# rapidsai/cudf

Hardware: NVIDIA H100
Metric: sort_by_key_rows_per_s (higher is better)
Workload: dtype int64

## Files before the change

### cudf_b200/csrc/radix_sort.cu

```cuda
#include "common.cuh"
#include "device_utils.cuh"

#include <algorithm>
#include <cmath>
#include <cstdlib>
#include <type_traits>

namespace b2 {
namespace {

constexpr int RADIX_BITS = 8;
constexpr int RADIX      = 256;
constexpr uint32_t FLAG_AGG  = 1u << 30;
constexpr uint32_t FLAG_INCL = 2u << 30;
constexpr uint32_t VAL_MASK  = (1u << 30) - 1;

struct pass_plan {
  int32_t trivial;
  int32_t key_src;
  int32_t key_dst;
  int32_t idx_src;
  int32_t idx_dst;
  int32_t last;
  int32_t hybrid;
// ... 289 lines not shown
  const void* key_bufs[3];
  int32_t* idx_bufs[3];
  sort_ctl* ctl;
  uint32_t* status;
  uint32_t* tile_counter;
  int64_t portion_start;
  uint32_t portion_n;
  int32_t pass;
  int32_t portion_parity;
  int32_t has_next_portion;
  int32_t kind;
  int32_t pairs;
  uint64_t desc_mask;
  int32_t keep_keys;
  const void* val_in;
  const void* range_splitters;
  void* const* range_key_dst;
  void* const* range_val_dst;
  int32_t range_parts;
  int32_t range_hash;
  uint32_t est_cap;
};

__host__ __device__ __forceinline__ unsigned range_hash_bucket(uint64_t twiddled_key, int parts)
{
  const uint64_t h = mix64(twiddled_key + 0x9E3779B97F4A7C15ull);
  return (unsigned)(((h >> 32) * (uint64_t)parts) >> 32);
}

__device__ __forceinline__ void cta_barrier(int nthreads)
{
// ... 117 lines not shown
               : "memory");
#else
  (void)mbar;
#endif
}

template <int THREADS, int IPT, int MIN_BLOCKS, bool BULK = false>
struct tile_shape {
  static constexpr int threads = THREADS, ipt = IPT, min_blocks = MIN_BLOCKS, tile = THREADS * IPT;
  static constexpr bool bulk = BULK;
};
using tile_384x16      = tile_shape<384, 16, 2>;
using tile_512x16      = tile_shape<512, 16, 1>;
using tile_512x20_bulk = tile_shape<512, 20, 1, true>;

template <typename UK, typename Shape, typename VT, bool CARRY, bool MIX, bool RANGE>
__global__ void __launch_bounds__(Shape::threads + 32 * LBW, Shape::min_blocks) onesweep_kernel(pass_args a)
{
  constexpr int THREADS = Shape::threads;
  constexpr int IPT     = Shape::ipt;
  constexpr bool BULK   = Shape::bulk;
  constexpr int TILE    = THREADS * IPT;
  constexpr int NWARPS = THREADS / 32;
  static_assert(THREADS >= RADIX, "need one ranking thread per digit");
  static_assert(!RANGE || (!MIX && !BULK), "the range-partition pass uses the plain key load");

  const pass_plan pl = a.ctl->plan[a.pass];
  if (pl.trivial) return;

  B2_DYNAMIC_SMEM(smem_raw);
  constexpr int STAGE_W = sizeof(UK) > sizeof(VT) ? sizeof(UK) : sizeof(VT);
// ... 2 lines not shown
  uint32_t* s_whist   = reinterpret_cast<uint32_t*>(smem_raw + (size_t)STAGE_W * TILE);
  uint32_t* s_bm      = s_whist + NWARPS * RADIX;
  uint32_t* s_off     = s_bm + NWARPS * RADIX;
  uint32_t* s_cnt     = s_off + RADIX;
  uint32_t* s_misc    = s_cnt + 2 * RADIX;
  UK* s_split         = reinterpret_cast<UK*>(s_misc + 16);
  void** s_kdst       = reinterpret_cast<void**>(s_split + RADIX);
  void** s_vdst       = s_kdst + RADIX;
  uint8_t* s_dig      = reinterpret_cast<uint8_t*>(s_vdst + RADIX);

  const int tid  = threadIdx.x;
  const int lane = tid & 31;
  const int warp = tid >> 5;
  const bool ranker = warp < NWARPS;

  if (tid == 0) s_misc[0] = atomicAdd(a.tile_counter, 1u);
  if constexpr (BULK && !EMU_BUILD) {
    if (tid == 0) mbar_init_one((uint32_t)__cvta_generic_to_shared(s_misc + 12));
  }
  if (ranker) {
#pragma unroll
    for (int j = 0; j < RADIX / 32; ++j) {
      s_whist[warp * RADIX + j * 32 + lane] = 0;
      s_bm[warp * RADIX + j * 32 + lane]    = 0;
    }
  }
  if constexpr (RANGE) {
    for (int i = tid; i < RADIX; i += THREADS + 32 * LBW) {
      s_split[i] = (!a.range_hash && i < a.range_parts - 1) ? static_cast<const UK*>(a.range_splitters)[i] : ~UK(0);
      s_kdst[i]  = i < a.range_parts ? a.range_key_dst[i] : nullptr;
      s_vdst[i]  = (CARRY && i < a.range_parts) ? a.range_val_dst[i] : nullptr;
    }
  }
  __syncthreads();
  const uint32_t tile = s_misc[0];
  const uint32_t tile_base = tile * (uint32_t)TILE;
  const uint32_t tile_n = min((uint32_t)TILE, a.portion_n - tile_base);
  const bool full = tile_n == (uint32_t)TILE;
  const uint32_t pad = (uint32_t)TILE - tile_n;
  const int shift = a.pass * RADIX_BITS;
  const UK desc = (UK)a.desc_mask;

  if (!ranker) {
    cta_barrier(THREADS + 32 * LBW);
    const int d0 = ((warp - NWARPS) * 32 + lane) * DPL;
    uint32_t cnt[DPL], loc[DPL], excl[DPL];
#pragma unroll
    for (int j = 0; j < DPL; j += 2) {
      const uint4 cs = *reinterpret_cast<const uint4*>(s_cnt + 2 * (d0 + j));
      cnt[j] = cs.x; loc[j] = cs.y; cnt[j + 1] = cs.z; loc[j + 1] = cs.w;
      excl[j] = 0; excl[j + 1] = 0;
    }
// ... 32 lines not shown
        const int n_ready   = __ffs(~usable) - 1;
        const int first_inc = (inc_all & usable) ? (__ffs(inc_all & usable) - 1) : LBT;
        const int take = min(n_ready, first_inc + 1);
        if (take == 0) { __nanosleep(40); continue; }
#pragma unroll
        for (int r = 0; r < LBT; ++r) {
          if (r < take) { excl[0] += v[r].x & VAL_MASK; excl[1] += v[r].y; excl[2] += v[r].z; excl[3] += v[r].w; }
        }
        done = first_inc < n_ready;
        t -= take;
      }
      publish(FLAG_INCL, excl[0] + cnt[0], excl[1] + cnt[1], excl[2] + cnt[2], excl[3] + cnt[3]);
    }
    const uint32_t* gb = &a.ctl->base[a.portion_parity][a.pass][d0];
    bool wants_end = a.has_next_portion != 0;
    if constexpr (MIX) wants_end = wants_end || a.est_cap != 0u;
    const bool last_of_portion = wants_end && tile_base + tile_n == a.portion_n;
#pragma unroll
    for (int j = 0; j < DPL; ++j) {
      const uint32_t g = gb[j];
      s_off[d0 + j] = g + excl[j] - loc[j];
      if (last_of_portion) a.ctl->base[a.portion_parity ^ 1][a.pass][d0 + j] = g + excl[j] + cnt[j];
    }
    cta_barrier(THREADS + 32 * LBW);
    return;
  }

  UK key[IPT];
  const uint32_t wbase = tile_base + warp * (32 * IPT) + lane;
  {
    const UK* src = static_cast<const UK*>(pl.key_src == 0 ? a.key_bufs[0] : (pl.key_src == 1 ? a.key_bufs[1] : a.key_bufs[2])) + a.portion_start;
    bool via_smem = false;
// ... 8 lines not shown
        } else {
          const uint32_t mbar = (uint32_t)__cvta_generic_to_shared(s_misc + 12);
          if (tid == 0) bulk_copy_to_smem(s_keys, src + tile_base, BYTES, mbar);
          mbar_wait_phase0(mbar);
        }
#pragma unroll
        for (int i = 0; i < IPT; ++i) key[i] = s_keys[warp * (32 * IPT) + i * 32 + lane];
      }
    } else if (full) {
#pragma unroll
      for (int i = 0; i < IPT; ++i) key[i] = ld_stream(src + wbase + i * 32);
    } else {
#pragma unroll
      for (int i = 0; i < IPT; ++i) {
        uint32_t e = wbase + i * 32;
        key[i] = e < a.portion_n ? ld_stream(src + e) : UK(0);
      }
    }
    if (pl.key_src == 0) {
#pragma unroll
      for (int i = 0; i < IPT; ++i) {
        if constexpr (MIX) key[i] = (UK)mix64((uint64_t)key[i]);
        else key[i] = twiddle_rt<UK>(key[i], a.kind, desc);
      }
    }
    if (!full) {
#pragma unroll
      for (int i = 0; i < IPT; ++i)
        if (wbase + i * 32 >= a.portion_n) key[i] = ~UK(0);
    }
  }

  auto digit_of = [&](UK k) -> unsigned {
    if constexpr (RANGE) {
      if (a.range_hash) return range_hash_bucket((uint64_t)k, a.range_parts);
      int lo = 0, hi = a.range_parts - 1;
      while (lo < hi) {
        const int mid = (lo + hi) >> 1;
        if (s_split[mid] <= k) lo = mid + 1;
        else hi = mid;
      }
      return (unsigned)lo;
    } else {
      return (unsigned)(k >> shift) & 255u;
    }
  };
  unsigned dg[RANGE ? IPT : 1];
  if constexpr (RANGE) {
#pragma unroll
    for (int i = 0; i < IPT; ++i) dg[i] = (wbase + i * 32 >= a.portion_n) ? (unsigned)(RADIX - 1) : digit_of(key[i]);
  }
  auto digit_at = [&](int i) -> unsigned {
    if constexpr (RANGE) return dg[i];
    else return (unsigned)(key[i] >> shift) & 255u;
  };
  uint32_t* my_hist = s_whist + warp * RADIX;
  const int distinct = warp_digit_counts<IPT>(digit_at, IPT, lane, my_hist);
  ranker_barrier(THREADS);

  uint32_t tstart = 0, count = 0;
  if (tid < RADIX) {
#pragma unroll
    for (int w = 0; w < NWARPS; ++w) {
      uint32_t c = s_whist[w * RADIX + tid];
      s_whist[w * RADIX + tid] = count;
      count += c;
    }
    const uint32_t padded = count;
    if (tid == RADIX - 1) count -= pad;
    uint32_t inc = warp_inclusive_sum(padded);
    if (lane == 31) s_misc[1 + warp] = inc;
    tstart = inc - padded;
  }
// ... 14 lines not shown
  warp_rank<IPT>(digit_at, IPT, distinct, lane, my_hist, s_bm + warp * RADIX, pos);
#pragma unroll
  for (int i = 0; i < IPT; ++i) s_keys[pos[i]] = key[i];
  if constexpr (RANGE) {
#pragma unroll
    for (int i = 0; i < IPT; ++i) s_dig[pos[i]] = (uint8_t)dg[i];
  }
  VT idx[IPT];
  if (a.pairs) {
    if (pl.idx_src < 0) {
      if constexpr (CARRY) {
        const VT* vsrc = static_cast<const VT*>(a.val_in) + a.portion_start;
#pragma unroll
        for (int i = 0; i < IPT; ++i) {
          const uint32_t e = wbase + i * 32;
          idx[i] = e < a.portion_n ? ld_stream(vsrc + e) : VT(0);
        }
      } else {
#pragma unroll
        for (int i = 0; i < IPT; ++i) idx[i] = (uint32_t)(a.portion_start + wbase + i * 32);
      }
    } else {
      const VT* isrc = reinterpret_cast<const VT*>(pl.idx_src == 0 ? a.idx_bufs[0] : (pl.idx_src == 1 ? a.idx_bufs[1] : a.idx_bufs[2])) + a.portion_start;
      if (full) {
#pragma unroll
        for (int i = 0; i < IPT; ++i) idx[i] = ld_stream(isrc + wbase + i * 32);
      } else {
#pragma unroll
        for (int i = 0; i < IPT; ++i) {
          uint32_t e = wbase + i * 32;
          idx[i] = e < a.portion_n ? ld_stream(isrc + e) : VT(0);
        }
      }
    }
  }
  cta_barrier(THREADS + 32 * LBW);

  const bool write_keys = !(a.pairs && pl.last) || a.keep_keys || pl.hybrid;
  UK* kdst = static_cast<UK*>(const_cast<void*>(pl.key_dst == 1 ? a.key_bufs[1] : a.key_bufs[2]));
  uint32_t dst[IPT];
  uint8_t dstd[RANGE ? IPT : 1];
#pragma unroll
  for (int j = 0; j < IPT; ++j) {
    const uint32_t q = j * THREADS + tid;
    UK k = s_keys[q];
    unsigned d;
    if constexpr (RANGE) d = s_dig[q];
    else d = (unsigned)(k >> shift) & 255u;
    dst[j] = s_off[d] + q;
    if constexpr (MIX) {
      if (a.est_cap != 0u && dst[j] >= (d + 1u) * a.est_cap) {
        if (q < tile_n) a.ctl->overflow = 1u;
        dst[j] = 0xFFFFFFFFu;
      }
    }
    if constexpr (RANGE) {
      dstd[j] = (uint8_t)d;
      if (q < tile_n) static_cast<UK*>(s_kdst[d])[dst[j]] = untwiddle_rt<UK>(k, a.kind, desc);
    } else if (write_keys && q < tile_n && (!MIX || dst[j] != 0xFFFFFFFFu)) {
      if (!a.pairs && pl.last && !pl.hybrid) k = untwiddle_rt<UK>(k, a.kind, desc);
      kdst[dst[j]] = k;
    }
  }
  if (a.pairs) {
    ranker_barrier(THREADS);
#pragma unroll
    for (int i = 0; i < IPT; ++i) s_vals[pos[i]] = idx[i];
    ranker_barrier(THREADS);
    VT* idst = reinterpret_cast<VT*>(pl.idx_dst == 0 ? a.idx_bufs[0] : (pl.idx_dst == 1 ? a.idx_bufs[1] : a.idx_bufs[2]));
#pragma unroll
    for (int j = 0; j < IPT; ++j) {
      const uint32_t q = j * THREADS + tid;
      if constexpr (RANGE) {
        if (q < tile_n) static_cast<VT*>(s_vdst[dstd[j]])[dst[j]] = s_vals[q];
      } else {
        if (q < tile_n && (!MIX || dst[j] != 0xFFFFFFFFu)) idst[dst[j]] = s_vals[q];
      }
    }
  }
}

template <typename UK, bool MIX = false>
__global__ void finalize_kernel(pass_args a, int64_t n, int raw, int pre_idx_buf, int carry_bytes)
{
  if (a.ctl->any_pass != 0) return;
  if (carry_bytes) {
    const int64_t stride = (int64_t)gridDim.x * blockDim.x;
    for (int64_t i = (int64_t)blockIdx.x * blockDim.x + threadIdx.x; i < n; i += stride) {
      if (carry_bytes == 8) reinterpret_cast<uint64_t*>(a.idx_bufs[0])[i] = static_cast<const uint64_t*>(a.val_in)[i];
      else reinterpret_cast<uint32_t*>(a.idx_bufs[0])[i] = static_cast<const uint32_t*>(a.val_in)[i];
      if (a.keep_keys && raw) {
// ... 153 lines not shown
  const bool bulk = (reinterpret_cast<uintptr_t>(g) % sizeof(T)) == 0 && s >= off && m + off >= PER;
  const int bulk_rows = bulk ? (m + off) / PER * PER : 0;
  if (bulk) {
    if constexpr (EMU_BUILD) {
      for (int q = threadIdx.x; q < bulk_rows; q += RANGE_THREADS) sdst[q] = g[q - off];
    } else {
      if (threadIdx.x == 0) bulk_copy_to_smem(sdst, g - off, (uint32_t)(sizeof(T) * bulk_rows), mbar);
    }
    for (int r = bulk_rows - off + (int)threadIdx.x; r < m; r += RANGE_THREADS) sdst[off + r] = g[r];
  } else {
    for (int q = threadIdx.x; q < m; q += RANGE_THREADS) sdst[q] = ld_stream(g + q);
  }
  return {bulk ? off : 0, bulk};
}

template <typename VT>
__global__ void __launch_bounds__(RANGE_THREADS, 1) range_sort_kernel(pass_args a, const uint32_t* __restrict__ bounds)
{
  using UK = uint64_t;
  B2_DYNAMIC_SMEM(smem_raw);
  uint32_t* s_misc = reinterpret_cast<uint32_t*>(smem_raw);
  UK* s_keys       = reinterpret_cast<UK*>(smem_raw + 128);
  VT* s_vals       = reinterpret_cast<VT*>(s_keys);
  uint32_t* s_cnt  = reinterpret_cast<uint32_t*>(s_keys + RANGE_CAP + 2);
  uint16_t* s_perm = reinterpret_cast<uint16_t*>(s_cnt + RANGE_BUCKETS);

  const int tid = threadIdx.x, lane = tid & 31, warp = tid >> 5;
  const int64_t s = bounds[blockIdx.x];
  const int m = (int)(bounds[blockIdx.x + 1] - s);
  if (m == 0) return;
  if (m > RANGE_CAP) {
    if (tid == 0) atomicOr(&a.ctl->overflow, 1u);
    return;
  }
  const UK* __restrict__ keys = static_cast<const UK*>(a.ctl->fix_key_buf == 1 ? a.key_bufs[1] : a.key_bufs[2]) + s;
  const VT* __restrict__ vin  = reinterpret_cast<const VT*>(a.ctl->fix_idx_buf == 1 ? a.idx_bufs[1] : a.idx_bufs[2]) + s;
  VT* __restrict__ vout = reinterpret_cast<VT*>(a.idx_bufs[0]) + s;
  UK* __restrict__ kout = static_cast<UK*>(const_cast<void*>(a.key_bufs[1])) + s;

  const uint64_t below = a.ctl->vary & ((1ull << a.ctl->range_shift) - 1);
  const uint32_t vhi = (uint32_t)(below >> 32), vlo = (uint32_t)below;
  const int top = vhi ? 64 - __clz((int)vhi) : (vlo ? 32 - __clz((int)vlo) : 0);
  const int want = m > 1 ? 32 - __clz(m - 1) : 0;
  const int nb = min(min(want, RANGE_BUCKET_BITS), top);
  const int bshift = top - nb;
  const uint32_t bmask = (1u << nb) - 1;
  const int lp = max(nb - 9, 0);
  const int per = 1 << lp;
  auto bucket = [&](UK k) { return (uint32_t)(k >> bshift) & bmask; };
  auto slot   = [&](uint32_t b) { return ((b & (uint32_t)(per - 1)) << 9) | (b >> lp); };

  const uint32_t mbar_k = EMU_BUILD ? 0u : (uint32_t)__cvta_generic_to_shared(s_misc);
  const uint32_t mbar_v = EMU_BUILD ? 0u : (uint32_t)__cvta_generic_to_shared(s_misc + 2);
// ... 198 lines not shown
    }
  }
}

int64_t portion_rows(int tile)
{
  static const int64_t lim = [] {
    const char* e = std::getenv("B2_SORT_PORTION");
    int64_t v = e ? std::atoll(e) : 0;
    if (v <= 0) v = (int64_t(1) << 30) - 16384;
    return v;
  }();
  return std::max<int64_t>(tile, lim / tile * tile);
}

template <typename UK, typename Shape, typename VT, bool CARRY, bool MIX, bool RANGE = false>
struct onesweep_passes {
  static constexpr int TILE = Shape::tile;
  static constexpr size_t SMEM = (sizeof(UK) > sizeof(VT) ? sizeof(UK) : sizeof(VT)) * (size_t)TILE +
                                 sizeof(uint32_t) * (2 * (Shape::threads / 32) * RADIX + 3 * RADIX + 16) +
                                 (RANGE ? (sizeof(UK) + 2 * sizeof(void*)) * RADIX + (size_t)TILE : 0);
  static constexpr size_t CTL_BYTES = (sizeof(sort_ctl) + 255) / 256 * 256;
  const int64_t n, plim, nportions;
  const size_t hist_bytes, cnt_bytes, head_bytes, status_per;
  dbuf work;

  onesweep_passes(int64_t rows, int passes, size_t hist, size_t tail_bytes, cudaStream_t stream)
    : n(rows), plim(portion_rows(TILE)), nportions((n + plim - 1) / plim), hist_bytes(hist),
      cnt_bytes((sizeof(uint32_t) * passes * nportions + 255) / 256 * 256), head_bytes(CTL_BYTES + hist_bytes + cnt_bytes + tail_bytes),
      status_per(sizeof(uint32_t) * RADIX * (size_t)((std::min(n, plim) + TILE - 1) / TILE)),
      work(head_bytes + status_per * passes * nportions, stream)
  {
    static std::atomic<uint64_t> attr_done{0};
    once_per_device(attr_done, [] {
      B2_CUDA_TRY(cudaFuncSetAttribute(onesweep_kernel<UK, Shape, VT, CARRY, MIX, RANGE>, cudaFuncAttributeMaxDynamicSharedMemorySize, (int)SMEM));
    });
  }
  sort_ctl* ctl() const { return work.as<sort_ctl>(); }
  uint32_t* hist() const { return reinterpret_cast<uint32_t*>(work.as<char>() + CTL_BYTES); }
  void* tail() const { return work.as<char>() + CTL_BYTES + hist_bytes + cnt_bytes; }
  void zero_head(cudaStream_t stream) const { B2_CUDA_TRY(cudaMemsetAsync(work.ptr, 0, head_bytes, stream)); }

  void run(pass_args& a, int slot, const char* scope, cudaStream_t stream) const
  {
    for (int64_t q = 0; q < nportions; ++q) {
      const int64_t start = q * plim;
      const int64_t pn = std::min(plim, n - start);
      const int64_t ntiles = (pn + TILE - 1) / TILE;
      a.portion_start = start;
      a.portion_n = (uint32_t)pn;
      a.portion_parity = (int)(q & 1);
      a.has_next_portion = q + 1 < nportions;
      a.status = reinterpret_cast<uint32_t*>(work.as<char>() + head_bytes + (size_t)(slot * nportions + q) * status_per);
      a.tile_counter = reinterpret_cast<uint32_t*>(work.as<char>() + CTL_BYTES + hist_bytes) + slot * nportions + q;
      B2_CUDA_TRY(cudaMemsetAsync(a.status, 0, sizeof(uint32_t) * RADIX * (size_t)ntiles, stream));
      prof_scope ps(scope, stream);
      B2_LAUNCH((onesweep_kernel<UK, Shape, VT, CARRY, MIX, RANGE>), (unsigned)ntiles, Shape::threads + 32 * LBW, SMEM, stream, a);
    }
  }
};

constexpr int64_t RANGE_MIN_ROWS = int64_t(1) << 27;
int range_env()
{
  static int v = [] {
    const char* e = std::getenv("B2_SORT_RANGE");
    return e ? (std::atoi(e) != 0 ? 1 : 0) : -1;
  }();
  return v;
}

int64_t hybrid_min_rows()
{
  static int64_t v = [] {
    const char* off = std::getenv("B2_SORT_HYBRID");
    if (off && std::atoi(off) == 0) return INT64_MAX;
    const char* e = std::getenv("B2_SORT_HYBRID_MIN");
    return e ? (int64_t)std::atoll(e) : (int64_t(1) << 16);
  }();
  return v;
}

template <typename UK, typename Shape, typename VT = uint32_t, bool CARRY = false, bool MIX = false>
void run_radix_cfg(const UK* raw_keys, UK* bufA, UK* bufB, int32_t* idx_out, int32_t* idx_tmp, int32_t* idx_tmp2, int pre_idx_buf, int64_t n,
                   int kind, bool descending, bool pairs, cudaStream_t stream, int first_pass = 0, int last_pass = 7,
                   bool keep_keys = false, const void* val_in = nullptr, uint32_t* top_digit_base_out = nullptr)
{
  constexpr int NP = sizeof(UK);
  const bool raw = raw_keys != nullptr;
  const UK desc_mask = descending ? ~UK(0) : UK(0);

  const onesweep_passes<UK, Shape, VT, CARRY, MIX> passes(n, NP, sizeof(uint32_t) * NP * RADIX, 0, stream);
  sort_ctl* const ctl = passes.ctl();
  uint32_t* const ghist = passes.hist();
  if constexpr (sizeof(UK) == 8 && !MIX) {
    static std::atomic<uint64_t> attr_done{0};
    once_per_device(attr_done, [] {
      B2_CUDA_TRY(cudaFuncSetAttribute(range_sort_kernel<VT>, cudaFuncAttributeMaxDynamicSharedMemorySize, (int)range_sort_smem()));
    });
  }

  bool try_hybrid = sizeof(UK) == 8 && !MIX && raw && first_pass == 0 && last_pass >= NP - 1 && !keep_keys && n >= hybrid_min_rows();
  const int force_range = range_env();
  bool try_range = try_hybrid && force_range != 0 && (force_range == 1 || n >= RANGE_MIN_ROWS);

// ... 107 lines not shown
    }
    try_hybrid = false;
  }
  if (pairs && raw && kind == (int)key_kind::FLOAT && descending) {
    B2_LAUNCH(reverse_nan_prefix_kernel, num_sms() * 4, 256, 0, stream, idx_out, &ctl->nan_count);
  }
  if (top_digit_base_out)
    B2_CUDA_TRY(cudaMemcpyAsync(top_digit_base_out, &ctl->base[0][NP - 1][0], sizeof(uint32_t) * RADIX, cudaMemcpyDeviceToDevice, stream));
}

template <typename UK>
using key_tile = std::conditional_t<sizeof(UK) == 8, tile_384x16, tile_512x16>;

template <typename UK>
void run_radix(const UK* raw_keys, UK* bufA, UK* bufB, int32_t* idx_out, int32_t* idx_tmp, int pre_idx_buf, int64_t n,
               int kind, bool descending, bool pairs, cudaStream_t stream, int32_t* idx_tmp2 = nullptr)
{
  run_radix_cfg<UK, key_tile<UK>>(raw_keys, bufA, bufB, idx_out, idx_tmp, idx_tmp2, pre_idx_buf, n, kind, descending, pairs, stream);
}

template void run_radix_cfg<uint64_t, tile_384x16>(const uint64_t*, uint64_t*, uint64_t*, int32_t*, int32_t*, int32_t*, int, int64_t, int, bool,
                                                   bool, cudaStream_t, int, int, bool, const void*, uint32_t*);

}

void radix_partition_top16_mix(const uint64_t* packed_keys, int64_t n, uint64_t* keys_out, int32_t* idx_out, cudaStream_t stream)
{
  dbuf b(sizeof(uint64_t) * n, stream), it(sizeof(int32_t) * n, stream);
  run_radix_cfg<uint64_t, tile_384x16, uint32_t, false, true>(packed_keys, keys_out, b.as<uint64_t>(), idx_out, it.as<int32_t>(), nullptr, 0,
                                                              n, (int)key_kind::UNSIGNED, false, true, stream, 6, 7, true);
}

void radix_partition_mix_carry(const uint64_t* keys, const void* vals, int val_bytes, int64_t n, uint64_t* mixed_keys_out, void* vals_out,
                               uint32_t* part_base, cudaStream_t stream)
{
  dbuf b(sizeof(uint64_t) * n, stream), vt((size_t)val_bytes * n, stream);
  if (val_bytes == 8)
// ... 19 lines not shown
      pl.idx_src = -1;
      pl.key_dst = 1;
      pl.idx_dst = 0;
      pl.last    = 1;
      pl.hybrid  = 0;
    }
    ctl->plan[d] = pl;
  }
  if (d == 0) {
    ctl->any_pass = 1;
    ctl->hybrid   = 0;
    ctl->overflow = 0;
  }
}

__global__ void __launch_bounds__(256) est_sample_kernel(const uint64_t* __restrict__ keys, int64_t n, int64_t stride, unsigned int* __restrict__ counts)
{
  __shared__ unsigned int sh[RADIX];
  sh[threadIdx.x] = 0;
  __syncthreads();
  const int64_t m = (n + stride - 1) / stride;
  for (int64_t i = (int64_t)blockIdx.x * blockDim.x + threadIdx.x; i < m; i += (int64_t)gridDim.x * blockDim.x)
    atomicAdd(&sh[(unsigned)(mix64(keys[i * stride]) >> 56)], 1u);
  __syncthreads();
  if (sh[threadIdx.x]) atomicAdd(&counts[threadIdx.x], sh[threadIdx.x]);
}

template <typename VT>
bool est_pass_impl(const uint64_t* keys, const void* vals, int64_t n, uint32_t cap, uint64_t* mixed_keys_out, void* vals_out, uint32_t* part_base,
                   uint32_t* part_end, cudaStream_t stream)
{
  constexpr int PASS = 7;
  const onesweep_passes<uint64_t, tile_384x16, VT, true, true> passes(n, 1, 0, 0, stream);
  sort_ctl* const ctl = passes.ctl();
  passes.zero_head(stream);
  B2_LAUNCH(est_plan_kernel, 1, RADIX, 0, stream, ctl, PASS, cap);
  pass_args a{};
  a.key_bufs[0] = keys;
  a.key_bufs[1] = mixed_keys_out;
  a.key_bufs[2] = mixed_keys_out;
// ... 19 lines not shown
}

uint32_t radix_partition_est_capacity(const uint64_t* keys, int64_t n, cudaStream_t stream)
{
  static const int64_t min_rows = [] {
    const char* e = std::getenv("B2_GROUPBY_EST_MIN");
    return e ? (int64_t)std::atoll(e) : (int64_t(1) << 22);
  }();
  if (n < min_rows || n > portion_rows(tile_384x16::tile)) return 0;
  if (const char* e = std::getenv("B2_GROUPBY_EST_CAP")) return (uint32_t)std::max(1, std::atoi(e));
  const int64_t want = int64_t(1) << 20;
  const int64_t stride = std::max<int64_t>(1, n / want);
  const int64_t m = (n + stride - 1) / stride;
  dbuf cnt(sizeof(unsigned int) * RADIX, stream);
  B2_CUDA_TRY(cudaMemsetAsync(cnt.ptr, 0, cnt.bytes, stream));
  B2_LAUNCH(est_sample_kernel, num_sms() * 4, 256, 0, stream, keys, n, stride, cnt.as<unsigned int>());
  unsigned int h[RADIX];
  B2_CUDA_TRY(cudaMemcpyAsync(h, cnt.ptr, sizeof(h), cudaMemcpyDeviceToHost, stream));
  B2_CUDA_TRY(cudaStreamSynchronize(stream));
  unsigned int mx = 0;
  for (int d = 0; d < RADIX; ++d) mx = std::max(mx, h[d]);
  const double cap = (double)(n / RADIX) * 1.25 + 4096.0;
  const double worst = ((double)mx + 5.0 * std::sqrt((double)mx) + 1.0) * ((double)n / (double)m);
  if (worst > cap || cap * RADIX >= 4.0e9) return 0;
  return (uint32_t)cap;
}

bool radix_partition_mix_carry_est(const uint64_t* keys, const void* vals, int val_bytes, int64_t n, uint32_t cap, uint64_t* mixed_keys_out,
                                   void* vals_out, uint32_t* part_base, uint32_t* part_end, cudaStream_t stream)
{
  if (val_bytes == 8) return est_pass_impl<uint64_t>(keys, vals, n, cap, mixed_keys_out, vals_out, part_base, part_end, stream);
// ... 96 lines not shown
}

void range_partition_scatter(const b2_column_view& keys, const b2_column_view* values, const void* splitters, int P, void* const* key_dst,
                             void* const* val_dst, cudaStream_t stream)
{
  if (keys.size == 0) return;
  if (values == nullptr) return range_scatter_impl<uint32_t, false>(keys, nullptr, splitters, P, key_dst, nullptr, stream);
  const int vw = type_width(values->type_id);
  const void* vin = static_cast<const char*>(values->data) + (size_t)values->offset * vw;
  if (vw == 8) range_scatter_impl<uint64_t, true>(keys, vin, splitters, P, key_dst, val_dst, stream);
  else range_scatter_impl<uint32_t, true>(keys, vin, splitters, P, key_dst, val_dst, stream);
}

namespace {

int kind_of(int32_t storage_id)
{
  if (is_float_id(storage_id)) return (int)key_kind::FLOAT;
  if (is_signed_id(storage_id)) return (int)key_kind::SIGNED;
  return (int)key_kind::UNSIGNED;
}

template <typename UK>
column_ptr sorted_order_single(const b2_column_view& col, bool ascending, bool nulls_before, cudaStream_t stream)
{
  const int64_t n = col.size;
  const int sid   = storage_type(col.type_id);
  const int kind  = kind_of(sid);
  auto out = make_column(B2_INT32, col.size, false, stream);
  const UK* data = static_cast<const UK*>(col.data) + col.offset;
  int32_t* out_idx = out->data.as<int32_t>();

  if (!has_nulls(col)) {
    dbuf a(sizeof(UK) * n, stream), b(sizeof(UK) > 1 ? sizeof(UK) * n : 0, stream), it(sizeof(int32_t) * n, stream);
    run_radix<UK>(data, a.as<UK>(), b.as<UK>(), out_idx, it.as<int32_t>(), 0, n, kind, !ascending, true, stream);
    return out;
  }
  const bool nulls_first = nulls_before != !ascending;
  const int64_t n_null  = col.null_count;
  const int64_t n_valid = n - n_null;
  const int64_t ntiles = (n + CP_ROWS - 1) / CP_ROWS;
  dbuf tv(sizeof(uint32_t) * (ntiles + 1), stream);
  B2_LAUNCH(valid_count_kernel, (unsigned)((ntiles + 7) / 8), CP_THREADS, 0, stream, col.null_mask, (int64_t)col.offset, n,
            tv.as<uint32_t>());
  B2_LAUNCH(scan_tiles_kernel, 1, 1024, 0, stream, tv.as<uint32_t>(), ntiles, tv.as<uint32_t>() + ntiles);
  dbuf a(sizeof(UK) * std::max<int64_t>(n_valid, 1), stream), b(sizeof(UK) * std::max<int64_t>(n_valid, 1), stream);
  dbuf it(sizeof(int32_t) * std::max<int64_t>(n_valid, 1), stream), it2(sizeof(int32_t) * std::max<int64_t>(n_valid, 1), stream);
  int32_t* valid_out = out_idx + (nulls_first ? n_null : 0);
  int32_t* null_out  = out_idx + (nulls_first ? 0 : n_valid);
  const UK desc_mask = ascending ? UK(0) : ~UK(0);
// ... 161 lines not shown
  return v;
}
bool sort_carry_applicable(const b2_column_view& keys, const b2_column_view& values, bool ascending)
{
  const int vw = type_width(values.type_id);
  const bool float_desc = is_float_id(storage_type(keys.type_id)) && !ascending;
  return sort_carry_enabled() && is_radix_sortable(keys) && !has_nulls(values) && (vw == 4 || vw == 8) && !float_desc &&
         keys.size == values.size && keys.size > 0;
}
column_ptr sort_by_key_carry(const b2_column_view& keys, const b2_column_view& values, bool ascending, cudaStream_t stream)
{
  const int64_t n = keys.size;
  const int kind = kind_of(storage_type(keys.type_id));
  auto out = make_column(values.type_id, (int32_t)n, false, stream);
  const int vw = type_width(values.type_id);
  dbuf vtmp((size_t)vw * n, stream);
  const void* vin = static_cast<const char*>(values.data) + (size_t)values.offset * vw;
  auto go = [&](auto ktag, auto vtag) {
    using UK = decltype(ktag);
    using VT = decltype(vtag);
    dbuf a(sizeof(UK) * n, stream), b(sizeof(UK) > 1 ? sizeof(UK) * n : 0, stream);
    using Shape = std::conditional_t<sizeof(UK) == 8 && sizeof(VT) == 8, tile_512x20_bulk, key_tile<UK>>;
    run_radix_cfg<UK, Shape, VT, true>(static_cast<const UK*>(keys.data) + keys.offset, a.as<UK>(), b.as<UK>(), out->data.as<int32_t>(),
                                       vtmp.as<int32_t>(), nullptr, 0, n, kind, !ascending, true, stream, 0, 7, false, vin);
  };
  auto by_key = [&](auto vtag) {
    switch (type_width(keys.type_id)) {
      case 1: go(uint8_t{}, vtag); break;
      case 2: go(uint16_t{}, vtag); break;
      case 4: go(uint32_t{}, vtag); break;
      default: go(uint64_t{}, vtag); break;
    }
  };
  if (vw == 8) by_key(uint64_t{}); else by_key(uint32_t{});
  return out;
}

column_ptr sort_single_column(const b2_column_view& col, bool ascending, cudaStream_t stream)
{
  const int64_t n = col.size;
  auto out = make_column(col.type_id, col.size, false, stream);
  if (n == 0) return out;
  const int kind = kind_of(storage_type(col.type_id));
  B2_EXPECTS(kind != (int)key_kind::FLOAT, B2_ERR_LOGIC, "keys-only radix path is for integer-like keys");
  auto run = [&](auto tag) {
    using UK = decltype(tag);
    dbuf tmp(sizeof(UK) > 1 ? sizeof(UK) * n : 0, stream);
    run_radix<UK>(static_cast<const UK*>(col.data) + col.offset, out->data.as<UK>(), tmp.as<UK>(), nullptr, nullptr, 0, n, kind,
                  !ascending, false, stream);
  };
  switch (type_width(col.type_id)) {
    case 1: run(uint8_t{}); break;
    case 2: run(uint16_t{}); break;
    case 4: run(uint32_t{}); break;
    case 8: run(uint64_t{}); break;
    default: B2_FAIL(B2_ERR_DATA_TYPE, "sort: unsupported key type");
  }
  return out;
}

}
```

Before: 22.72 billion.

## Add sampled-capacity two-pass MSD radix tier with range sort for 64-bit keys

Adds an estimated-capacity path for 64-bit keys. A sampling kernel builds histograms of the top two digits and picks a per-bucket capacity. Only the top two radix passes then run, scattering into padded fixed-offset buckets, and a range_sort kernel sorts each of the 65536 segments, replacing the six remaining onesweep passes. This costs extra memory (padded buffers), a host sync for sampling plus a later overflow check with fallback, and more kernels.

```diff
diff --git a/cudf_b200/csrc/radix_sort.cu b/cudf_b200/csrc/radix_sort.cu
--- a/cudf_b200/csrc/radix_sort.cu
+++ b/cudf_b200/csrc/radix_sort.cu
@@ -327,7 +327,10 @@
   uint64_t desc_mask;
   int32_t keep_keys;
   const void* val_in;
-  const void* range_splitters;
+  union {
+    const void* range_splitters;
+    const uint2* est_tiles;
+  };
   void* const* range_key_dst;
   void* const* range_val_dst;
   int32_t range_parts;
@@ -475,7 +478,7 @@
 using tile_512x16      = tile_shape<512, 16, 1>;
 using tile_512x20_bulk = tile_shape<512, 20, 1, true>;
 
-template <typename UK, typename Shape, typename VT, bool CARRY, bool MIX, bool RANGE>
+template <typename UK, typename Shape, typename VT, bool CARRY, bool MIX, bool RANGE, bool EST = false>
 __global__ void __launch_bounds__(Shape::threads + 32 * LBW, Shape::min_blocks) onesweep_kernel(pass_args a)
 {
   constexpr int THREADS = Shape::threads;
@@ -508,7 +511,19 @@
   const int warp = tid >> 5;
   const bool ranker = warp < NWARPS;
 
-  if (tid == 0) s_misc[0] = atomicAdd(a.tile_counter, 1u);
+  if (tid == 0) {
+    const uint32_t t = atomicAdd(a.tile_counter, 1u);
+    s_misc[0] = t;
+    if constexpr (EST) {
+      s_misc[10] = 0;
+      s_misc[11] = 0;
+      if (a.est_tiles != nullptr) {
+        const uint2 e = a.est_tiles[t];
+        s_misc[9]  = e.x;
+        s_misc[14] = e.y;
+      }
+    }
+  }
   if constexpr (BULK && !EMU_BUILD) {
     if (tid == 0) mbar_init_one((uint32_t)__cvta_generic_to_shared(s_misc + 12));
   }
@@ -528,8 +543,17 @@
   }
   __syncthreads();
   const uint32_t tile = s_misc[0];
-  const uint32_t tile_base = tile * (uint32_t)TILE;
-  const uint32_t tile_n = min((uint32_t)TILE, a.portion_n - tile_base);
+  uint32_t tile_base = tile * (uint32_t)TILE;
+  uint32_t tile_n = min((uint32_t)TILE, a.portion_n - tile_base);
+  uint32_t nlim = a.portion_n;
+  if constexpr (EST) {
+    if (a.est_tiles != nullptr) {
+      if (s_misc[14] == 0) return;
+      tile_base = s_misc[9];
+      tile_n    = s_misc[14] & 0x7fffffffu;
+      nlim      = tile_base + tile_n;
+    }
+  }
   const bool full = tile_n == (uint32_t)TILE;
   const uint32_t pad = (uint32_t)TILE - tile_n;
   const int shift = a.pass * RADIX_BITS;
@@ -592,8 +616,12 @@
     }
     const uint32_t* gb = &a.ctl->base[a.portion_parity][a.pass][d0];
     bool wants_end = a.has_next_portion != 0;
-    if constexpr (MIX) wants_end = wants_end || a.est_cap != 0u;
-    const bool last_of_portion = wants_end && tile_base + tile_n == a.portion_n;
+    if constexpr (MIX || EST) wants_end = wants_end || a.est_cap != 0u;
+    bool last_tile = tile_base + tile_n == a.portion_n;
+    if constexpr (EST) {
+      if (a.est_tiles != nullptr) last_tile = (s_misc[14] >> 31) != 0u;
+    }
+    const bool last_of_portion = wants_end && last_tile;
 #pragma unroll
     for (int j = 0; j < DPL; ++j) {
       const uint32_t g = gb[j];
@@ -632,7 +660,7 @@
 #pragma unroll
       for (int i = 0; i < IPT; ++i) {
         uint32_t e = wbase + i * 32;
-        key[i] = e < a.portion_n ? ld_stream(src + e) : UK(0);
+        key[i] = e < nlim ? ld_stream(src + e) : UK(0);
       }
     }
     if (pl.key_src == 0) {
@@ -645,7 +673,22 @@
     if (!full) {
 #pragma unroll
       for (int i = 0; i < IPT; ++i)
-        if (wbase + i * 32 >= a.portion_n) key[i] = ~UK(0);
+        if (wbase + i * 32 >= nlim) key[i] = ~UK(0);
+    }
+    if constexpr (EST) {
+      if (pl.key_src == 0) {
+        const UK k0 = twiddle_rt<UK>(static_cast<const UK*>(a.key_bufs[0])[0], a.kind, desc);
+        uint64_t v = 0;
+#pragma unroll
+        for (int i = 0; i < IPT; ++i)
+          if (wbase + i * 32 < nlim) v |= (uint64_t)(key[i] ^ k0);
+        const uint32_t lo = __reduce_or_sync(0xffffffffu, (uint32_t)v);
+        const uint32_t hi = __reduce_or_sync(0xffffffffu, (uint32_t)(v >> 32));
+        if (lane == 0 && (lo | hi)) {
+          atomicOr(&s_misc[10], lo);
+          atomicOr(&s_misc[11], hi);
+        }
+      }
     }
   }
 
@@ -666,7 +709,7 @@
   unsigned dg[RANGE ? IPT : 1];
   if constexpr (RANGE) {
 #pragma unroll
-    for (int i = 0; i < IPT; ++i) dg[i] = (wbase + i * 32 >= a.portion_n) ? (unsigned)(RADIX - 1) : digit_of(key[i]);
+    for (int i = 0; i < IPT; ++i) dg[i] = (wbase + i * 32 >= nlim) ? (unsigned)(RADIX - 1) : digit_of(key[i]);
   }
   auto digit_at = [&](int i) -> unsigned {
     if constexpr (RANGE) return dg[i];
@@ -675,6 +718,12 @@
   uint32_t* my_hist = s_whist + warp * RADIX;
   const int distinct = warp_digit_counts<IPT>(digit_at, IPT, lane, my_hist);
   ranker_barrier(THREADS);
+  if constexpr (EST) {
+    if (tid == 0 && pl.key_src == 0) {
+      const unsigned long long v = ((unsigned long long)s_misc[11] << 32) | s_misc[10];
+      if (v) atomicOr(&a.ctl->vary, v);
+    }
+  }
 
   uint32_t tstart = 0, count = 0;
   if (tid < RADIX) {
@@ -719,7 +768,7 @@
 #pragma unroll
         for (int i = 0; i < IPT; ++i) {
           const uint32_t e = wbase + i * 32;
-          idx[i] = e < a.portion_n ? ld_stream(vsrc + e) : VT(0);
+          idx[i] = e < nlim ? ld_stream(vsrc + e) : VT(0);
         }
       } else {
 #pragma unroll
@@ -734,7 +783,7 @@
 #pragma unroll
         for (int i = 0; i < IPT; ++i) {
           uint32_t e = wbase + i * 32;
-          idx[i] = e < a.portion_n ? ld_stream(isrc + e) : VT(0);
+          idx[i] = e < nlim ? ld_stream(isrc + e) : VT(0);
         }
       }
     }
@@ -753,7 +802,7 @@
     if constexpr (RANGE) d = s_dig[q];
     else d = (unsigned)(k >> shift) & 255u;
     dst[j] = s_off[d] + q;
-    if constexpr (MIX) {
+    if constexpr (MIX || EST) {
       if (a.est_cap != 0u && dst[j] >= (d + 1u) * a.est_cap) {
         if (q < tile_n) a.ctl->overflow = 1u;
         dst[j] = 0xFFFFFFFFu;
@@ -762,7 +811,7 @@
     if constexpr (RANGE) {
       dstd[j] = (uint8_t)d;
       if (q < tile_n) static_cast<UK*>(s_kdst[d])[dst[j]] = untwiddle_rt<UK>(k, a.kind, desc);
-    } else if (write_keys && q < tile_n && (!MIX || dst[j] != 0xFFFFFFFFu)) {
+    } else if (write_keys && q < tile_n && (!(MIX || EST) || dst[j] != 0xFFFFFFFFu)) {
       if (!a.pairs && pl.last && !pl.hybrid) k = untwiddle_rt<UK>(k, a.kind, desc);
       kdst[dst[j]] = k;
     }
@@ -779,7 +828,7 @@
       if constexpr (RANGE) {
         if (q < tile_n) static_cast<VT*>(s_vdst[dstd[j]])[dst[j]] = s_vals[q];
       } else {
-        if (q < tile_n && (!MIX || dst[j] != 0xFFFFFFFFu)) idst[dst[j]] = s_vals[q];
+        if (q < tile_n && (!(MIX || EST) || dst[j] != 0xFFFFFFFFu)) idst[dst[j]] = s_vals[q];
       }
     }
   }
@@ -963,7 +1012,36 @@
   return {bulk ? off : 0, bulk};
 }
 
-template <typename VT>
+__global__ void __launch_bounds__(RADIX) range_est_bounds_kernel(pass_args a, uint32_t cap, uint32_t* __restrict__ est)
+{
+  __shared__ uint32_t s_lb[RADIX + 1];
+  __shared__ uint32_t s_wsum[RADIX / 32];
+  constexpr int R = RADIX * RADIX;
+  const int d7 = blockIdx.x, d6 = threadIdx.x;
+  const uint64_t* __restrict__ keys = static_cast<const uint64_t*>(a.ctl->fix_key_buf == 1 ? a.key_bufs[1] : a.key_bufs[2]);
+  auto count = [&](int e) { return min(a.ctl->base[1][7][e] - (uint32_t)e * cap, cap); };
+  const uint32_t before = warp_sum(d6 < d7 ? count(d6) : 0u);
+  if ((d6 & 31) == 0) s_wsum[d6 >> 5] = before;
+  const uint32_t w0 = (uint32_t)d7 * cap, wn = count(d7);
+  uint32_t lo = 0, hi = wn;
+  while (lo < hi) {
+    const uint32_t mid = (lo + hi) >> 1;
+    if ((int)((keys[w0 + mid] >> 48) & 255u) < d6) lo = mid + 1;
+    else hi = mid;
+  }
+  s_lb[d6] = lo;
+  if (d6 == 0) s_lb[RADIX] = wn;
+  __syncthreads();
+  uint32_t dense = 0;
+  for (int w = 0; w < RADIX / 32; ++w) dense += s_wsum[w];
+  const uint32_t end = s_lb[d6 + 1];
+  const int i = d7 * RADIX + d6;
+  est[i]         = w0 + lo;
+  est[R + i]     = end > lo ? end - lo : 0u;
+  est[2 * R + i] = dense + lo;
+}
+
+template <typename VT, bool EST = false>
 __global__ void __launch_bounds__(RANGE_THREADS, 1) range_sort_kernel(pass_args a, const uint32_t* __restrict__ bounds)
 {
   using UK = uint64_t;
@@ -976,7 +1054,14 @@
 
   const int tid = threadIdx.x, lane = tid & 31, warp = tid >> 5;
   const int64_t s = bounds[blockIdx.x];
-  const int m = (int)(bounds[blockIdx.x + 1] - s);
+  int m;
+  int64_t o = s;
+  if constexpr (EST) {
+    m = (int)bounds[gridDim.x + blockIdx.x];
+    o = bounds[2 * gridDim.x + blockIdx.x];
+  } else {
+    m = (int)(bounds[blockIdx.x + 1] - s);
+  }
   if (m == 0) return;
   if (m > RANGE_CAP) {
     if (tid == 0) atomicOr(&a.ctl->overflow, 1u);
@@ -984,8 +1069,8 @@
   }
   const UK* __restrict__ keys = static_cast<const UK*>(a.ctl->fix_key_buf == 1 ? a.key_bufs[1] : a.key_bufs[2]) + s;
   const VT* __restrict__ vin  = reinterpret_cast<const VT*>(a.ctl->fix_idx_buf == 1 ? a.idx_bufs[1] : a.idx_bufs[2]) + s;
-  VT* __restrict__ vout = reinterpret_cast<VT*>(a.idx_bufs[0]) + s;
-  UK* __restrict__ kout = static_cast<UK*>(const_cast<void*>(a.key_bufs[1])) + s;
+  VT* __restrict__ vout = reinterpret_cast<VT*>(a.idx_bufs[0]) + o;
+  UK* __restrict__ kout = static_cast<UK*>(const_cast<void*>(a.key_bufs[1])) + o;
 
   const uint64_t below = a.ctl->vary & ((1ull << a.ctl->range_shift) - 1);
   const uint32_t vhi = (uint32_t)(below >> 32), vlo = (uint32_t)below;
@@ -1214,7 +1299,7 @@
   return std::max<int64_t>(tile, lim / tile * tile);
 }
 
-template <typename UK, typename Shape, typename VT, bool CARRY, bool MIX, bool RANGE = false>
+template <typename UK, typename Shape, typename VT, bool CARRY, bool MIX, bool RANGE = false, bool EST = false>
 struct onesweep_passes {
   static constexpr int TILE = Shape::tile;
   static constexpr size_t SMEM = (sizeof(UK) > sizeof(VT) ? sizeof(UK) : sizeof(VT)) * (size_t)TILE +
@@ -1225,15 +1310,16 @@
   const size_t hist_bytes, cnt_bytes, head_bytes, status_per;
   dbuf work;
 
-  onesweep_passes(int64_t rows, int passes, size_t hist, size_t tail_bytes, cudaStream_t stream)
+  onesweep_passes(int64_t rows, int passes, size_t hist, size_t tail_bytes, cudaStream_t stream, int extra_tiles = 0)
     : n(rows), plim(portion_rows(TILE)), nportions((n + plim - 1) / plim), hist_bytes(hist),
       cnt_bytes((sizeof(uint32_t) * passes * nportions + 255) / 256 * 256), head_bytes(CTL_BYTES + hist_bytes + cnt_bytes + tail_bytes),
-      status_per(sizeof(uint32_t) * RADIX * (size_t)((std::min(n, plim) + TILE - 1) / TILE)),
+      status_per(sizeof(uint32_t) * RADIX * (size_t)((std::min(n, plim) + TILE - 1) / TILE + extra_tiles)),
       work(head_bytes + status_per * passes * nportions, stream)
   {
     static std::atomic<uint64_t> attr_done{0};
     once_per_device(attr_done, [] {
-      B2_CUDA_TRY(cudaFuncSetAttribute(onesweep_kernel<UK, Shape, VT, CARRY, MIX, RANGE>, cudaFuncAttributeMaxDynamicSharedMemorySize, (int)SMEM));
+      B2_CUDA_TRY(cudaFuncSetAttribute(onesweep_kernel<UK, Shape, VT, CARRY, MIX, RANGE, EST>, cudaFuncAttributeMaxDynamicSharedMemorySize,
+                                       (int)SMEM));
     });
   }
   sort_ctl* ctl() const { return work.as<sort_ctl>(); }
@@ -1241,12 +1327,12 @@
   void* tail() const { return work.as<char>() + CTL_BYTES + hist_bytes + cnt_bytes; }
   void zero_head(cudaStream_t stream) const { B2_CUDA_TRY(cudaMemsetAsync(work.ptr, 0, head_bytes, stream)); }
 
-  void run(pass_args& a, int slot, const char* scope, cudaStream_t stream) const
+  void run(pass_args& a, int slot, const char* scope, cudaStream_t stream, int extra_tiles = 0) const
   {
     for (int64_t q = 0; q < nportions; ++q) {
       const int64_t start = q * plim;
       const int64_t pn = std::min(plim, n - start);
-      const int64_t ntiles = (pn + TILE - 1) / TILE;
+      const int64_t ntiles = (pn + TILE - 1) / TILE + extra_tiles;
       a.portion_start = start;
       a.portion_n = (uint32_t)pn;
       a.portion_parity = (int)(q & 1);
@@ -1255,7 +1341,7 @@
       a.tile_counter = reinterpret_cast<uint32_t*>(work.as<char>() + CTL_BYTES + hist_bytes) + slot * nportions + q;
       B2_CUDA_TRY(cudaMemsetAsync(a.status, 0, sizeof(uint32_t) * RADIX * (size_t)ntiles, stream));
       prof_scope ps(scope, stream);
-      B2_LAUNCH((onesweep_kernel<UK, Shape, VT, CARRY, MIX, RANGE>), (unsigned)ntiles, Shape::threads + 32 * LBW, SMEM, stream, a);
+      B2_LAUNCH((onesweep_kernel<UK, Shape, VT, CARRY, MIX, RANGE, EST>), (unsigned)ntiles, Shape::threads + 32 * LBW, SMEM, stream, a);
     }
   }
 };
@@ -1281,14 +1367,132 @@
   return v;
 }
 
+__global__ void range_est_plan_kernel(sort_ctl* ctl, uint32_t cap)
+{
+  const int d = threadIdx.x;
+  ctl->base[0][6][d] = (uint32_t)d * cap;
+  ctl->base[0][7][d] = (uint32_t)d * cap;
+  if (d < 8) {
+    pass_plan pl{};
+    pl.trivial = d < 6;
+    if (d >= 6) {
+      pl.key_src = d == 6 ? 0 : 1;
+      pl.key_dst = d == 6 ? 1 : 2;
+      pl.idx_src = d == 6 ? -1 : 2;
+      pl.idx_dst = d == 6 ? 2 : 1;
+      pl.last    = d == 7;
+      pl.hybrid  = 1;
+    }
+    ctl->plan[d] = pl;
+  }
+  if (d == 0) {
+    ctl->any_pass    = 2;
+    ctl->hybrid      = 1;
+    ctl->range       = 1;
+    ctl->range_shift = 48;
+    ctl->range_bits  = 16;
+    ctl->fix_shift   = 48;
+    ctl->fix_key_buf = 2;
+    ctl->fix_idx_buf = 1;
+    ctl->overflow    = 0;
+  }
+}
+
+__global__ void range_est_tiles_kernel(const sort_ctl* ctl, uint32_t cap, int tile, uint2* __restrict__ tiles)
+{
+  __shared__ uint32_t s_wsum[RADIX / 32];
+  const int d = threadIdx.x;
+  const uint32_t cnt = min(ctl->base[1][6][d] - (uint32_t)d * cap, cap);
+  const uint32_t nt = (cnt + (uint32_t)tile - 1) / (uint32_t)tile;
+  const uint32_t inc = warp_inclusive_sum(nt);
+  if ((d & 31) == 31) s_wsum[d >> 5] = inc;
+  __syncthreads();
+  uint32_t first = inc - nt, total = 0;
+  for (int w = 0; w < RADIX / 32; ++w) {
+    first += w < (d >> 5) ? s_wsum[w] : 0u;
+    total += s_wsum[w];
+  }
+  for (uint32_t k = 0; k < nt; ++k) {
+    const uint32_t off = k * (uint32_t)tile;
+    const uint32_t t = first + k;
+    tiles[t] = make_uint2((uint32_t)d * cap + off, min((uint32_t)tile, cnt - off) | (t + 1 == total ? 0x80000000u : 0u));
+  }
+}
+
+template <typename UK, typename Shape, typename VT, bool CARRY>
+bool run_est_range(const UK* raw_keys, UK* keys_out, UK* k1, UK* k2, int32_t* idx_out, int32_t* v1, int32_t* v2, int64_t n, uint32_t cap,
+                   int kind, UK desc_mask, bool pairs, const void* val_in, cudaStream_t stream)
+{
+  static_assert(sizeof(UK) == 8, "the estimated-base range tier sorts 64-bit keys");
+  constexpr int TILE = Shape::tile;
+  const int64_t ntiles = (n + TILE - 1) / TILE + RADIX;
+  const size_t table_bytes = (sizeof(uint2) * ntiles + 255) / 256 * 256;
+  const onesweep_passes<UK, Shape, VT, CARRY, false, false, true> passes(n, 2, 0, table_bytes, stream, RADIX);
+  {
+    static std::atomic<uint64_t> attr_done{0};
+    once_per_device(attr_done, [] {
+      B2_CUDA_TRY(cudaFuncSetAttribute(range_sort_kernel<VT, true>, cudaFuncAttributeMaxDynamicSharedMemorySize, (int)range_sort_smem()));
+    });
+  }
+  sort_ctl* const ctl = passes.ctl();
+  uint2* const tiles = static_cast<uint2*>(passes.tail());
+  passes.zero_head(stream);
+  B2_LAUNCH(range_est_plan_kernel, 1, RADIX, 0, stream, ctl, cap);
+  pass_args a{};
+  a.key_bufs[0] = raw_keys;
+  a.key_bufs[1] = k1;
+  a.key_bufs[2] = k2;
+  a.idx_bufs[0] = idx_out;
+  a.idx_bufs[1] = v2;
+  a.idx_bufs[2] = v1;
+  a.ctl = ctl;
+  a.kind = kind;
+  a.pairs = pairs ? 1 : 0;
+  a.val_in = val_in;
+  a.desc_mask = (uint64_t)desc_mask;
+  a.est_cap = cap;
+  a.pass = 6;
+  passes.run(a, 0, "onesweep", stream);
+  B2_LAUNCH(range_est_tiles_kernel, 1, RADIX, 0, stream, (const sort_ctl*)ctl, cap, TILE, tiles);
+  a.pass = 7;
+  a.est_tiles = tiles;
+  passes.run(a, 1, "onesweep", stream, RADIX);
+  a.key_bufs[1] = keys_out;
+  dbuf bounds(sizeof(uint32_t) * 3 * RADIX * RADIX, stream);
+  {
+    prof_scope ps("range_bounds", stream);
+    B2_LAUNCH(range_est_bounds_kernel, RADIX, RADIX, 0, stream, a, cap, bounds.as<uint32_t>());
+  }
+  {
+    prof_scope ps("segment_fix", stream);
+    B2_LAUNCH((range_sort_kernel<VT, true>), RADIX * RADIX, RANGE_THREADS, range_sort_smem(), stream, a, bounds.as<const uint32_t>());
+  }
+  uint32_t overflow = 0;
+  B2_CUDA_TRY(cudaMemcpyAsync(&overflow, &ctl->overflow, sizeof(overflow), cudaMemcpyDeviceToHost, stream));
+  B2_CUDA_TRY(cudaStreamSynchronize(stream));
+  return overflow == 0;
+}
+
 template <typename UK, typename Shape, typename VT = uint32_t, bool CARRY = false, bool MIX = false>
 void run_radix_cfg(const UK* raw_keys, UK* bufA, UK* bufB, int32_t* idx_out, int32_t* idx_tmp, int32_t* idx_tmp2, int pre_idx_buf, int64_t n,
                    int kind, bool descending, bool pairs, cudaStream_t stream, int first_pass = 0, int last_pass = 7,
-                   bool keep_keys = false, const void* val_in = nullptr, uint32_t* top_digit_base_out = nullptr)
+                   bool keep_keys = false, const void* val_in = nullptr, uint32_t* top_digit_base_out = nullptr, uint32_t est_cap = 0,
+                   void* est_buf = nullptr)
 {
   constexpr int NP = sizeof(UK);
   const bool raw = raw_keys != nullptr;
   const UK desc_mask = descending ? ~UK(0) : UK(0);
+
+  if constexpr (sizeof(UK) == 8 && !MIX) {
+    if (est_cap != 0 && raw && first_pass == 0 && last_pass >= NP - 1 && !keep_keys) {
+      const bool done =
+        pairs ? run_est_range<UK, Shape, VT, CARRY>(raw_keys, bufA, bufA, bufB, idx_out, static_cast<int32_t*>(est_buf), idx_tmp, n, est_cap,
+                                                    kind, desc_mask, true, val_in, stream)
+              : run_est_range<UK, Shape, VT, CARRY>(raw_keys, bufA, static_cast<UK*>(est_buf), bufB, nullptr, nullptr, nullptr, n, est_cap,
+                                                    kind, desc_mask, false, val_in, stream);
+      if (done) return;
+    }
+  }
 
   const onesweep_passes<UK, Shape, VT, CARRY, MIX> passes(n, NP, sizeof(uint32_t) * NP * RADIX, 0, stream);
   sort_ctl* const ctl = passes.ctl();
@@ -1426,13 +1630,15 @@
 
 template <typename UK>
 void run_radix(const UK* raw_keys, UK* bufA, UK* bufB, int32_t* idx_out, int32_t* idx_tmp, int pre_idx_buf, int64_t n,
-               int kind, bool descending, bool pairs, cudaStream_t stream, int32_t* idx_tmp2 = nullptr)
-{
-  run_radix_cfg<UK, key_tile<UK>>(raw_keys, bufA, bufB, idx_out, idx_tmp, idx_tmp2, pre_idx_buf, n, kind, descending, pairs, stream);
+               int kind, bool descending, bool pairs, cudaStream_t stream, int32_t* idx_tmp2 = nullptr, uint32_t est_cap = 0,
+               void* est_buf = nullptr)
+{
+  run_radix_cfg<UK, key_tile<UK>>(raw_keys, bufA, bufB, idx_out, idx_tmp, idx_tmp2, pre_idx_buf, n, kind, descending, pairs, stream, 0, 7,
+                                  false, nullptr, nullptr, est_cap, est_buf);
 }
 
 template void run_radix_cfg<uint64_t, tile_384x16>(const uint64_t*, uint64_t*, uint64_t*, int32_t*, int32_t*, int32_t*, int, int64_t, int, bool,
-                                                   bool, cudaStream_t, int, int, bool, const void*, uint32_t*);
+                                                   bool, cudaStream_t, int, int, bool, const void*, uint32_t*, uint32_t, void*);
 
 }
 
@@ -1482,16 +1688,27 @@
   }
 }
 
-__global__ void __launch_bounds__(256) est_sample_kernel(const uint64_t* __restrict__ keys, int64_t n, int64_t stride, unsigned int* __restrict__ counts)
-{
-  __shared__ unsigned int sh[RADIX];
-  sh[threadIdx.x] = 0;
+template <bool MIX = true>
+__global__ void __launch_bounds__(256) est_sample_kernel(const uint64_t* __restrict__ keys, int64_t n, int64_t stride, unsigned int* __restrict__ counts,
+                                                         int kind = 0, uint64_t desc_mask = 0)
+{
+  constexpr int NC = MIX ? 1 : 2;
+  __shared__ unsigned int sh[NC * RADIX];
+  for (int c = 0; c < NC; ++c) sh[c * RADIX + threadIdx.x] = 0;
   __syncthreads();
   const int64_t m = (n + stride - 1) / stride;
-  for (int64_t i = (int64_t)blockIdx.x * blockDim.x + threadIdx.x; i < m; i += (int64_t)gridDim.x * blockDim.x)
-    atomicAdd(&sh[(unsigned)(mix64(keys[i * stride]) >> 56)], 1u);
+  for (int64_t i = (int64_t)blockIdx.x * blockDim.x + threadIdx.x; i < m; i += (int64_t)gridDim.x * blockDim.x) {
+    if constexpr (MIX) {
+      atomicAdd(&sh[(unsigned)(mix64(keys[i * stride]) >> 56)], 1u);
+    } else {
+      const uint64_t k = twiddle_rt<uint64_t>(keys[i * stride], kind, desc_mask);
+      atomicAdd(&sh[(unsigned)(k >> 56)], 1u);
+      atomicAdd(&sh[RADIX + (unsigned)((k >> 48) & 255u)], 1u);
+    }
+  }
   __syncthreads();
-  if (sh[threadIdx.x]) atomicAdd(&counts[threadIdx.x], sh[threadIdx.x]);
+  for (int c = 0; c < NC; ++c)
+    if (sh[c * RADIX + threadIdx.x]) atomicAdd(&counts[c * RADIX + threadIdx.x], sh[c * RADIX + threadIdx.x]);
 }
 
 template <typename VT>
@@ -1541,7 +1758,7 @@
   const int64_t m = (n + stride - 1) / stride;
   dbuf cnt(sizeof(unsigned int) * RADIX, stream);
   B2_CUDA_TRY(cudaMemsetAsync(cnt.ptr, 0, cnt.bytes, stream));
-  B2_LAUNCH(est_sample_kernel, num_sms() * 4, 256, 0, stream, keys, n, stride, cnt.as<unsigned int>());
+  B2_LAUNCH((est_sample_kernel<true>), num_sms() * 4, 256, 0, stream, keys, n, stride, cnt.as<unsigned int>(), 0, (uint64_t)0);
   unsigned int h[RADIX];
   B2_CUDA_TRY(cudaMemcpyAsync(h, cnt.ptr, sizeof(h), cudaMemcpyDeviceToHost, stream));
   B2_CUDA_TRY(cudaStreamSynchronize(stream));
@@ -1668,6 +1885,60 @@
 
 namespace {
 
+int est_env()
+{
+  static int v = [] {
+    const char* e = std::getenv("B2_SORT_EST");
+    return e ? (std::atoi(e) != 0 ? 1 : 0) : -1;
+  }();
+  return v;
+}
+
+template <typename UK>
+uint32_t est_range_capacity(const UK* raw_keys, int64_t n, int kind, bool descending, bool pairs, int tile, cudaStream_t stream)
+{
+  if constexpr (sizeof(UK) != 8) {
+    return 0;
+  } else {
+    const int force = est_env();
+    if (force == 0 || n < 2 || n > portion_rows(tile)) return 0;
+    if (pairs && kind == (int)key_kind::FLOAT && descending) return 0;
+    if (range_env() == 0 || hybrid_min_rows() == INT64_MAX) return 0;
+    if (force != 1 && (n < RANGE_MIN_ROWS || n < hybrid_min_rows())) return 0;
+    if (const char* e = std::getenv("B2_SORT_EST_CAP")) return (uint32_t)std::max(1, std::atoi(e));
+    const int64_t stride = std::max<int64_t>(1, n >> 20);
+    const int64_t m = (n + stride - 1) / stride;
+    dbuf cnt(sizeof(unsigned int) * 2 * RADIX, stream);
+    B2_CUDA_TRY(cudaMemsetAsync(cnt.ptr, 0, cnt.bytes, stream));
+    {
+      prof_scope ps("est_sample", stream);
+      const int grid = (int)std::max<int64_t>(1, std::min<int64_t>((m + 255) / 256, num_sms() * 4));
+      B2_LAUNCH((est_sample_kernel<false>), grid, 256, 0, stream, reinterpret_cast<const uint64_t*>(raw_keys), n, stride, cnt.as<unsigned int>(),
+                kind, (uint64_t)(descending ? ~UK(0) : UK(0)));
+    }
+    unsigned int h[2 * RADIX];
+    B2_CUDA_TRY(cudaMemcpyAsync(h, cnt.ptr, sizeof(h), cudaMemcpyDeviceToHost, stream));
+    B2_CUDA_TRY(cudaStreamSynchronize(stream));
+    unsigned int mx[2] = {0, 0};
+    double coll[2] = {0.0, 0.0};
+    for (int c = 0; c < 2; ++c)
+      for (int d = 0; d < RADIX; ++d) {
+        mx[c] = std::max(mx[c], h[c * RADIX + d]);
+        const double f = (double)h[c * RADIX + d] / (double)m;
+        coll[c] += f * f;
+      }
+    if (mx[0] >= (unsigned)m || mx[1] >= (unsigned)m) return 0;
+    const double e = (double)n * coll[0] * coll[1];
+    if (e + 5.0 * std::sqrt(e) > (double)RANGE_CAP) return 0;
+    const double top = (double)std::max(mx[0], mx[1]);
+    const double worst = (top + 5.0 * std::sqrt(top) + 1.0) * ((double)n / (double)m);
+    if (worst > (double)(n / RADIX) * 1.25 + 4096.0) return 0;
+    const uint64_t cap = ((uint64_t)std::ceil(worst) + 15) / 16 * 16;
+    if (cap * RADIX >= 4000000000ull) return 0;
+    return (uint32_t)cap;
+  }
+}
+
 int kind_of(int32_t storage_id)
 {
   if (is_float_id(storage_id)) return (int)key_kind::FLOAT;
@@ -1686,8 +1957,11 @@
   int32_t* out_idx = out->data.as<int32_t>();
 
   if (!has_nulls(col)) {
-    dbuf a(sizeof(UK) * n, stream), b(sizeof(UK) > 1 ? sizeof(UK) * n : 0, stream), it(sizeof(int32_t) * n, stream);
-    run_radix<UK>(data, a.as<UK>(), b.as<UK>(), out_idx, it.as<int32_t>(), 0, n, kind, !ascending, true, stream);
+    const uint32_t cap = est_range_capacity<UK>(data, n, kind, !ascending, true, key_tile<UK>::tile, stream);
+    const int64_t rows = cap ? std::max<int64_t>(n, (int64_t)RADIX * cap) : n;
+    dbuf a(sizeof(UK) * rows, stream), b(sizeof(UK) > 1 ? sizeof(UK) * rows : 0, stream), it(sizeof(int32_t) * rows, stream);
+    dbuf ev(cap ? sizeof(int32_t) * RADIX * (size_t)cap : 0, stream);
+    run_radix<UK>(data, a.as<UK>(), b.as<UK>(), out_idx, it.as<int32_t>(), 0, n, kind, !ascending, true, stream, nullptr, cap, ev.ptr);
     return out;
   }
   const bool nulls_first = nulls_before != !ascending;
@@ -1879,15 +2153,18 @@
   const int kind = kind_of(storage_type(keys.type_id));
   auto out = make_column(values.type_id, (int32_t)n, false, stream);
   const int vw = type_width(values.type_id);
-  dbuf vtmp((size_t)vw * n, stream);
   const void* vin = static_cast<const char*>(values.data) + (size_t)values.offset * vw;
   auto go = [&](auto ktag, auto vtag) {
     using UK = decltype(ktag);
     using VT = decltype(vtag);
-    dbuf a(sizeof(UK) * n, stream), b(sizeof(UK) > 1 ? sizeof(UK) * n : 0, stream);
     using Shape = std::conditional_t<sizeof(UK) == 8 && sizeof(VT) == 8, tile_512x20_bulk, key_tile<UK>>;
-    run_radix_cfg<UK, Shape, VT, true>(static_cast<const UK*>(keys.data) + keys.offset, a.as<UK>(), b.as<UK>(), out->data.as<int32_t>(),
-                                       vtmp.as<int32_t>(), nullptr, 0, n, kind, !ascending, true, stream, 0, 7, false, vin);
+    const UK* kin = static_cast<const UK*>(keys.data) + keys.offset;
+    const uint32_t cap = est_range_capacity<UK>(kin, n, kind, !ascending, true, Shape::tile, stream);
+    const int64_t rows = cap ? std::max<int64_t>(n, (int64_t)RADIX * cap) : n;
+    dbuf vtmp((size_t)vw * rows, stream), a(sizeof(UK) * rows, stream), b(sizeof(UK) > 1 ? sizeof(UK) * rows : 0, stream);
+    dbuf ev(cap ? (size_t)vw * RADIX * cap : 0, stream);
+    run_radix_cfg<UK, Shape, VT, true>(kin, a.as<UK>(), b.as<UK>(), out->data.as<int32_t>(), vtmp.as<int32_t>(), nullptr, 0, n, kind, !ascending,
+                                       true, stream, 0, 7, false, vin, nullptr, cap, ev.ptr);
   };
   auto by_key = [&](auto vtag) {
     switch (type_width(keys.type_id)) {
@@ -1910,9 +2187,11 @@
   B2_EXPECTS(kind != (int)key_kind::FLOAT, B2_ERR_LOGIC, "keys-only radix path is for integer-like keys");
   auto run = [&](auto tag) {
     using UK = decltype(tag);
-    dbuf tmp(sizeof(UK) > 1 ? sizeof(UK) * n : 0, stream);
-    run_radix<UK>(static_cast<const UK*>(col.data) + col.offset, out->data.as<UK>(), tmp.as<UK>(), nullptr, nullptr, 0, n, kind,
-                  !ascending, false, stream);
+    const UK* kin = static_cast<const UK*>(col.data) + col.offset;
+    const uint32_t cap = est_range_capacity<UK>(kin, n, kind, !ascending, false, key_tile<UK>::tile, stream);
+    const int64_t rows = cap ? std::max<int64_t>(n, (int64_t)RADIX * cap) : n;
+    dbuf tmp(sizeof(UK) > 1 ? sizeof(UK) * rows : 0, stream), ev(cap ? sizeof(UK) * RADIX * (size_t)cap : 0, stream);
+    run_radix<UK>(kin, out->data.as<UK>(), tmp.as<UK>(), nullptr, nullptr, 0, n, kind, !ascending, false, stream, nullptr, cap, ev.ptr);
   };
   switch (type_width(col.type_id)) {
     case 1: run(uint8_t{}); break;
```

After: 24.41 billion (median of 6 runs). +7.4%, better.
